# zacz08/ADM

Hardware: AMD Instinct MI355X
Metric: train images/sec (CIFAR-10 32x32 uncond DDM UNet, 1 optimizer step/iter) + 10-step sample images/sec (higher is better)
Workload: dtype f32; 1 GPU; BASELINE configs[1]: CIFAR-10 32x32 uncond two-decoder DhariwalUNet (216M params), bs=128/GPU fp32, ddm_const schedule, dropout 0.1, loss_simple (LPIPS term needs unfetchable VGG16 weights), clip 1.0 + AdamW + EMA(every 8); global_batch=128, image=3x32x32, parallelism=dp1, valid=True

## Files before the change

adm_amd/csrc/conv_wino2d_x6.hip:

```cpp
#include "common.h"
#include "split_format.h"
#include <type_traits>

#ifndef X6_TL
#define X6_TL 0
#endif
#ifndef X6_SHARE
#define X6_SHARE 0
#endif
#ifndef X6_ABL
#define X6_ABL 0
#endif

namespace {

struct X6P {
  const float* x; const unsigned short* w; const float* bias; const float* res; float* y;
  int Mt, N, H, W, Hh, Wh, Cin, ldx, ldy, ldr, wrows, tilesN, xbytes, wbytes, plane;
  int splitk, chunks_per_split; float* ws;
  int ybytes, rbytes;
  int up;
  const float* amax_x; float wscale;
};

typedef __attribute__((address_space(3))) void x6_lds_void;
constexpr int X6P_T = 64, X6N = 64, X6K = 16;
[[maybe_unused]] constexpr int X6_A_STAGE = 4 * 3 * X6P_T * X6K;
[[maybe_unused]] constexpr int X6_B_STAGE = 4 * 3 * X6N * X6K;
template <int FMT, int NB = 2> struct X6Fmt {
  static constexpr int TERMS = split_terms(FMT);
  static constexpr int NT = 32 * NB;
  static constexpr int CONS = 2 * NB;
  static constexpr int THREADS = (CONS + 4) * 64;
  static constexpr int A_STAGE = 4 * TERMS * X6P_T * X6K;
  static constexpr int B_STAGE = 4 * TERMS * NT * X6K;
  static constexpr int DMA_PER_WAVE = 2 * TERMS;
  static constexpr int RB = NB > 2 ? 3 : 4;
  static constexpr int PD = NB > 2 ? 3 : 4;
};
constexpr int X6_RA = 2;

__device__ __forceinline__ f32x4 sub4(f32x4 a, f32x4 b) { return a - b; }
__device__ __forceinline__ f32x16 sub16(f32x16 a, f32x16 b) { return a - b; }

__device__ __forceinline__ void h3_store(const f32x4 (&e)[4], unsigned short* la, float s) {
  if (X6_ABL & 2) return;
  const f32x4 v[4] = {plain_sub4(e[0], e[2]), plain_add4(e[1], e[2]), plain_sub4(e[2], e[1]), plain_sub4(e[1], e[3])};
#pragma unroll
  for (int ex = 0; ex < 4; ++ex) {
    u32x2 t0, t1;
    split2_quad(v[ex], s, t0, t1);
    *reinterpret_cast<u32x2*>(la + (ex * 2 + 0) * X6P_T * X6K) = t0;
    *reinterpret_cast<u32x2*>(la + (ex * 2 + 1) * X6P_T * X6K) = t1;
  }
}

__device__ __forceinline__ void x6_store(const f32x4 (&e)[4], unsigned short* la) {
  if (X6_ABL & 2) return;
  const f32x4 v[4] = {plain_sub4(e[0], e[2]), plain_add4(e[1], e[2]), plain_sub4(e[2], e[1]), plain_sub4(e[1], e[3])};
#pragma unroll
  for (int ex = 0; ex < 4; ++ex) {
    u32x2 t0, t1, t2;
    split3_quad(v[ex], t0, t1, t2);
    *reinterpret_cast<u32x2*>(la + (ex * 3 + 0) * X6P_T * X6K) = t0;
    *reinterpret_cast<u32x2*>(la + (ex * 3 + 1) * X6P_T * X6K) = t1;
    *reinterpret_cast<u32x2*>(la + (ex * 3 + 2) * X6P_T * X6K) = t2;
  }
}

#ifndef X6_KB_N
#define X6_KB_N 4
#endif
constexpr int X6_KB = X6_KB_N;
struct X6Seq {
  int k0, len, ey, cc, skip2;
  __device__ __forceinline__ void init(int chunks, int up) { k0 = 0; len = min(X6_KB, chunks); ey = 0; cc = 0; skip2 = up; }
  __device__ __forceinline__ int chunk() const { return k0 + cc; }
  __device__ __forceinline__ bool done() const { return len <= 0; }
  __device__ __forceinline__ void next(int chunks) {
    if (++cc == len) {
      cc = 0;
      ++ey;
      if (skip2 && ey == 2) ++ey;
      if (ey == 4) { ey = 0; k0 += len; len = min(X6_KB, chunks - k0); }
    }
  }
};

template <int FMT, int NB>
__global__ __launch_bounds__((2 * NB + 4) * 64) void wino2d_x6_kernel(X6P p) {
  using F = X6Fmt<FMT, NB>;
  constexpr int TERMS = F::TERMS;
  float sa = 1.f, inv_scale = 1.f;
  if (FMT) { sa = split_scale(adm_amax_read(p.amax_x)); inv_scale = 1.f / (sa * p.wscale); }
  extern __shared__ __attribute__((aligned(16))) unsigned short smem6[];
  unsigned short* As = smem6;
  unsigned short* Bs = smem6 + X6_RA * F::A_STAGE;
  const int tid = threadIdx.x, lane = tid & 63, hw_wid = tid >> 6;
  const bool producer = hw_wid >= F::CONS;
  const int wid = producer ? hw_wid - F::CONS : hw_wid;
  const int bid = adm_xcd_remap(blockIdx.x, gridDim.x);
  const int tilesM = gridDim.x / p.tilesN;
  const int tm = bid % tilesM, tn = bid / tilesM;
  const int mt0 = tm * X6P_T, n0 = tn * F::NT;
  constexpr unsigned OOB = 0x80000000u;

  const int c_begin = (p.splitk > 1) ? (int)blockIdx.y * p.chunks_per_split : 0;
  const int chunks = (p.splitk > 1) ? min(p.chunks_per_split, (p.Cin >> 4) - c_begin) : (p.Cin >> 4);
  const int S = (p.up ? 3 : 4) * chunks;

  if (producer) {
    const __amdgpu_buffer_rsrc_t rs_x = __builtin_amdgcn_make_buffer_rsrc(const_cast<float*>(p.x), 0, p.xbytes, 0x00020000);
    const int ptid = wid * 64 + lane;
    const int pl = ptid >> 2, aq = ptid & 3;
    unsigned a_base = 0, colmask = 0, rowmask = 0;
    bool take_l = false, take_r = false;
    {
      const int t = mt0 + pl;
      if (t < p.Mt) {
        const int xp = t % p.Wh;
        const int u = t / p.Wh;
        const int ty = u % p.Hh, b = u / p.Hh;
        a_base = p.up ? (unsigned)((((long)b * p.Hh + ty) * p.Wh + xp) * p.ldx + aq * 4) * 4u
                      : (unsigned)((((long)b * p.H + 2 * ty) * p.W + 2 * xp) * p.ldx + aq * 4) * 4u;
        colmask = (xp > 0 ? 1u : 0u) | 6u | (2 * xp + 2 < p.W ? 8u : 0u);
        rowmask = (ty > 0 ? 1u : 0u) | 6u | (2 * ty + 2 < p.H ? 8u : 0u);
        if (X6_SHARE && !p.up) {
          take_l = xp > 0 && (pl & 15) != 0;
          take_r = xp + 1 < p.Wh && (pl & 15) != 15 && t + 1 < p.Mt;
          if (take_l) colmask &= ~1u;
          if (take_r) colmask &= ~8u;
        }
      }
    }
    unsigned short* la = As + pl * X6K + ((((aq >> 1) ^ (pl >> 3)) & 1) << 3) + (aq & 1) * 4;
    X6Seq ld; ld.init(chunks, p.up);
    unsigned a_voff[2][4];
    int voff_ey = -1;
    auto set_rows = [&]() {
      const int ey = ld.ey;
      const int iA = (ey == 0) ? 0 : 1, iB = (ey == 3) ? 3 : 2;
      const bool live = !ld.done();
      const bool vA = ((rowmask >> iA) & 1u) && live, vB = ((rowmask >> iB) & 1u) && live;
      const int offA = (p.up ? ((iA + 1) >> 1) - 1 : iA - 1) * (p.up ? p.Wh : p.W) * p.ldx * 4;
      const int offB = (p.up ? ((iB + 1) >> 1) - 1 : iB - 1) * (p.up ? p.Wh : p.W) * p.ldx * 4;
#pragma unroll
      for (int j = 0; j < 4; ++j) {
        const bool cv = (colmask >> j) & 1u;
        const int cj = (p.up ? ((j + 1) >> 1) - 1 : j - 1) * p.ldx * 4;
        a_voff[0][j] = (vA && cv) ? a_base + (unsigned)(offA + cj) : OOB;
        a_voff[1][j] = (vB && cv) ? a_base + (unsigned)(offB + cj) : OOB;
      }
      voff_ey = live ? ey : 4;
    };
    constexpr int D = F::PD;
    f32x4 dA[D][4], dB[D][4];
    int set_ey[D];
    auto issue = [&](int d) {
      if (voff_ey != (ld.done() ? 4 : ld.ey)) set_rows();
      const int soff = (c_begin + ld.chunk()) << 6;
#pragma unroll
      for (int j = 0; j < 4; ++j) {
        if (X6_ABL & 1) { dA[d][j] = f32x4{1.f, 2.f, 3.f, (float)soff}; dB[d][j] = f32x4{0.5f, 0.25f, (float)j, 1.f}; continue; }
        dA[d][j] = __builtin_bit_cast(f32x4, __builtin_amdgcn_raw_buffer_load_b128(rs_x, (int)a_voff[0][j], soff, 0));
        dB[d][j] = __builtin_bit_cast(f32x4, __builtin_amdgcn_raw_buffer_load_b128(rs_x, (int)a_voff[1][j], soff, 0));
      }
      set_ey[d] = ld.ey;
      if (!ld.done()) ld.next(chunks);
    };
    auto store = [&](int d, int slot) {
      f32x4 e[4];
      if (set_ey[d] == 1) {
#pragma unroll
        for (int j = 0; j < 4; ++j) e[j] = plain_add4(dA[d][j], dB[d][j]);
      } else if (set_ey[d] == 2) {
#pragma unroll
        for (int j = 0; j < 4; ++j) e[j] = plain_sub4(dB[d][j], dA[d][j]);
      } else {
#pragma unroll
        for (int j = 0; j < 4; ++j) e[j] = plain_sub4(dA[d][j], dB[d][j]);
      }
      if (X6_SHARE && !p.up) {
        f32x4 el, er;
#pragma unroll
        for (int i = 0; i < 4; ++i) { el[i] = __shfl_up(e[2][i], 4, 64); er[i] = __shfl_down(e[1][i], 4, 64); }
        if (take_l) e[0] = el;
        if (take_r) e[3] = er;
      }
      if (FMT) h3_store(e, la + slot * F::A_STAGE, sa);
      else x6_store(e, la + slot * F::A_STAGE);
    };
#pragma unroll
    for (int d = 0; d < D; ++d) issue(d);
    __builtin_amdgcn_sched_barrier(0);
    constexpr int TRIP = (D & 1) ? 2 * D : D;
    for (int t = 0; t < S; t += TRIP) {
#pragma unroll
      for (int k = 0; k < TRIP; ++k) {
        const int d = k % D;
        if (t + k < S) {
          const bool tl = X6_TL && p.ws && blockIdx.x == 0 && tid == F::CONS * 64 && t + k < 48;
          unsigned long long* TL = reinterpret_cast<unsigned long long*>(p.ws) + 1024 + (t + k) * 4;
          if (tl) TL[0] = __builtin_readcyclecounter();
          store(d, k & 1);
          __builtin_amdgcn_sched_barrier(0);
          if (tl) { asm volatile("s_waitcnt lgkmcnt(0)" ::: "memory"); TL[1] = __builtin_readcyclecounter(); }
          issue(d);
          __builtin_amdgcn_sched_barrier(0);
          if (tl) TL[2] = __builtin_readcyclecounter();
          adm_lds_barrier();
          if (tl) TL[3] = __builtin_readcyclecounter();
        }
      }
    }
    return;
  }

  const __amdgpu_buffer_rsrc_t rs_w = __builtin_amdgcn_make_buffer_rsrc(const_cast<unsigned short*>(p.w), 0, p.wbytes, 0x00020000);
  const int wm = wid / NB, wn = wid % NB;
  const int lr = lane & 31, lh = lane >> 5;
  if (p.splitk > 1) {
    p.y = p.ws + (long)blockIdx.y * ((long)p.Mt * 4) * p.N;
    p.ldy = p.N; p.bias = nullptr; p.res = nullptr;
    const long sb = (long)p.Mt * 4 * p.N * 4;
    p.ybytes = sb < (1L << 31) ? (int)sb : 0;
  }
  constexpr int QW = F::DMA_PER_WAVE;
  unsigned b_voff[QW];
#pragma unroll
  for (int i = 0; i < QW; ++i) {
    const int q = wid * QW + i, pt = q / NB;
    const int row = (q % NB) * 32 + (lane >> 1);
    const int n = n0 + row;
    const int half = (lane ^ (row >> 3)) & 1;
    b_voff[i] = (n < p.wrows) ? (unsigned)((((long)pt * p.wrows + n) * 16 + half * 8) * 2) : OOB;
  }
  X6Seq lb; lb.init(chunks, p.up);
  int ld_slot = 0;
  auto issue_b = [&]() {
    const int kb = ((lb.ey * (p.Cin >> 4) + c_begin + lb.chunk()) * (4 * TERMS) * p.wrows) << 5;
    unsigned short* dst = Bs + ld_slot * F::B_STAGE + (wid * QW) * 512;
    if (!(X6_ABL & 4)) {
#pragma unroll
      for (int i = 0; i < QW; ++i)
        __builtin_amdgcn_raw_ptr_buffer_load_lds(rs_w, (x6_lds_void*)(dst + i * 512), 16, (int)b_voff[i], kb, 0, 0);
    }
    lb.next(chunks);
    if (++ld_slot == F::RB) ld_slot = 0;
  };

  f32x16 acc[4];
  f32x16 Y[2][2];
#pragma unroll
  for (int a = 0; a < 2; ++a)
#pragma unroll
    for (int b = 0; b < 2; ++b)
#pragma unroll
      for (int r = 0; r < 16; ++r) Y[a][b][r] = 0.f;
  const int a_foff = (wm * 32 + lr) * X6K + ((lh ^ (lr >> 3)) & 1) * 8;
  const int b_foff = (wn * 32 + lr) * X6K + ((lh ^ (lr >> 3)) & 1) * 8;
  const f32x16 zero = {0.f, 0.f, 0.f, 0.f, 0.f, 0.f, 0.f, 0.f, 0.f, 0.f, 0.f, 0.f, 0.f, 0.f, 0.f, 0.f};

  X6Seq cs; cs.init(chunks, p.up);
  int slot_b = 0;
#pragma unroll
  for (int i = 0; i < F::RB - 1; ++i) issue_b();
  for (int t = 0; t < S; ++t) {
    const bool tl = X6_TL && p.ws && blockIdx.x == 0 && tid == 0 && t < 48;
    unsigned long long* TL = reinterpret_cast<unsigned long long*>(p.ws) + t * 4;
    if (tl) TL[0] = __builtin_readcyclecounter();
    if (F::RB == 4 && t + 2 < S) { if (FMT) asm volatile("s_waitcnt vmcnt(8) lgkmcnt(0)\n\ts_barrier" ::: "memory"); else asm volatile("s_waitcnt vmcnt(12) lgkmcnt(0)\n\ts_barrier" ::: "memory"); }
    else if (t + 1 < S) { if (FMT) asm volatile("s_waitcnt vmcnt(4) lgkmcnt(0)\n\ts_barrier" ::: "memory"); else asm volatile("s_waitcnt vmcnt(6) lgkmcnt(0)\n\ts_barrier" ::: "memory"); }
    else asm volatile("s_waitcnt vmcnt(0) lgkmcnt(0)\n\ts_barrier" ::: "memory");
    if (tl) TL[1] = __builtin_readcyclecounter();
    if (t + F::RB - 1 < S) issue_b();
    const unsigned short* Ab = As + (t & 1) * F::A_STAGE + a_foff;
    const unsigned short* Bb = Bs + slot_b * F::B_STAGE + b_foff;
    if (++slot_b == F::RB) slot_b = 0;
    const bool first = cs.cc == 0;
    u32x4 fa[NB > 2 ? 1 : 2][TERMS], fb[NB > 2 ? 1 : 2][TERMS];
    auto frag = [&](int xi, int set) {
#pragma unroll
      for (int k = 0; k < TERMS; ++k) {
        if (X6_ABL & 16) {
          fa[set][k] = u32x4{0x3f803f80u, (unsigned)t, 0x3f803f80u, (unsigned)xi};
          fb[set][k] = u32x4{0x3f003f00u, (unsigned)k, 0x3f003f00u, (unsigned)lane};
          continue;
        }
        fa[set][k] = *reinterpret_cast<const u32x4*>(Ab + (xi * TERMS + k) * X6P_T * X6K);
        fb[set][k] = *reinterpret_cast<const u32x4*>(Bb + (xi * TERMS + k) * F::NT * X6K);
      }
    };
    auto products = [&](auto first_tag) {
      if (NB > 2) {
#pragma unroll
        for (int xi = 0; xi < 4; ++xi) {
          frag(xi, 0);
          if (X6_ABL & 8) continue;
          const f16x8 a0 = __builtin_bit_cast(f16x8, fa[0][0]), a1 = __builtin_bit_cast(f16x8, fa[0][1]);
          const f16x8 b0 = __builtin_bit_cast(f16x8, fb[0][0]), b1 = __builtin_bit_cast(f16x8, fb[0][1]);
          f32x16 c;
          if (decltype(first_tag)::value) asm volatile("v_mfma_f32_32x32x16_f16 %0, %1, %2, 0" : "=&v"(c) : "v"(a0), "v"(b1));
          else c = __builtin_amdgcn_mfma_f32_32x32x16_f16(a0, b1, acc[xi], 0, 0, 0);
          c = __builtin_amdgcn_mfma_f32_32x32x16_f16(a1, b0, c, 0, 0, 0);
          acc[xi] = __builtin_amdgcn_mfma_f32_32x32x16_f16(a0, b0, c, 0, 0, 0);
        }
        return;
      }
      frag(0, 0);
#pragma unroll
      for (int xi = 0; xi < 4; ++xi) {
        const int cur = xi & 1;
        if (xi < 3) frag(xi + 1, cur ^ 1);
        __builtin_amdgcn_sched_barrier(0);
        if (X6_ABL & 8) continue;
        const f32x16 c0 = decltype(first_tag)::value ? zero : acc[xi];
// ... 107 lines not shown
      p.y[px * p.ldy + n] = y0;
      p.y[(px + 1) * p.ldy + n] = y1;
    }
  }
}

__global__ void split3_kernel(const float* __restrict__ src, unsigned short* __restrict__ dst, int rows, int cols) {
  const long per = (long)rows * cols, total = per * 16;
  for (long i = blockIdx.x * (long)blockDim.x + threadIdx.x; i < total; i += (long)gridDim.x * blockDim.x) {
    const int img = (int)(i / per);
    const long rc = i - img * per;
    const int n = (int)(rc / cols), c = (int)(rc - (long)n * cols);
    split3_store(src[i], dst + wino_image_offset(3, img >> 2, img & 3, rows, cols, n, c), split_term_stride(rows));
  }
}

__global__ void split2_kernel(const float* __restrict__ src, unsigned short* __restrict__ dst, int rows, int cols, float scale,
                              int* __restrict__ overflow) {
  const long per = (long)rows * cols, total = per * 16;
  bool bad = false;
  for (long i = blockIdx.x * (long)blockDim.x + threadIdx.x; i < total; i += (long)gridDim.x * blockDim.x) {
    const int img = (int)(i / per);
    const long rc = i - img * per;
    const int n = (int)(rc / cols), c = (int)(rc - (long)n * cols);
    const float a = src[i] * scale;
    bad |= split_f16_overflow(a);
    split2_store(a, dst + wino_image_offset(2, img >> 2, img & 3, rows, cols, n, c), split_term_stride(rows));
  }
  if (bad && overflow) *overflow = 1;
}

}

extern "C" int adm_split3_bf16(const float* src, void* dst, int rows, int cols, hipStream_t stream) {
  if (!src || !dst || rows <= 0 || cols <= 0 || (cols & 15)) return ADM_EINVAL;
  const long total = (long)rows * cols * 16;
  const int grid = (int)((total + 255) / 256 > 4096 ? 4096 : (total + 255) / 256);
  hipLaunchKernelGGL(split3_kernel, dim3(grid), dim3(256), 0, stream, src, static_cast<unsigned short*>(dst), rows, cols);
  ADM_CHECK_LAUNCH();
  return ADM_OK;
}

extern "C" int adm_split2_f16(const float* src, void* dst, int rows, int cols, float scale, int* overflow, hipStream_t stream) {
  if (!src || !dst || rows <= 0 || cols <= 0 || (cols & 15) || !(scale > 0.f)) return ADM_EINVAL;
  const long total = (long)rows * cols * 16;
  const int grid = (int)((total + 255) / 256 > 4096 ? 4096 : (total + 255) / 256);
  hipLaunchKernelGGL(split2_kernel, dim3(grid), dim3(256), 0, stream, src, static_cast<unsigned short*>(dst), rows, cols, scale, overflow);
  ADM_CHECK_LAUNCH();
  return ADM_OK;
}

static int g_h3_wide = -1;
extern "C" int adm_wino2d_h3_wide(int v) { const int old = g_h3_wide; g_h3_wide = v; return old; }

static int wino2d_x6_launch(const float* x, const void* wq6, const float* bias, const float* res, float* y, float* ws, long ws_floats,
                            int B, int H, int W, int Cin, int ldx, int N, int wrows, int ldy, int ldr, int up, hipStream_t stream,
                            const float* amax_x = nullptr, float wscale = 0.f) {
  const bool h3 = amax_x != nullptr;
  if (!x || !wq6 || !y || B <= 0 || H < 2 || W < 2 || (W & 1) || (H & 1)) return ADM_EINVAL;
  if ((Cin & 31) || (ldx & 3) || N <= 0 || wrows < N) return ADM_EINVAL;
  if (((uintptr_t)x | (uintptr_t)wq6) & 15) return ADM_EINVAL;
  X6P p;
  p.x = x; p.w = static_cast<const unsigned short*>(wq6); p.bias = bias; p.res = res; p.y = y;
  const long Mt = (long)B * (H / 2) * (W / 2);
  const long xb = (long)B * H * W * ldx * 4 / (up ? 4 : 1), wb = (h3 ? 32L : 48L) * wrows * Cin * 2;
  if (h3 && !(wscale > 0.f)) return ADM_EINVAL;
  if (Mt >= (1L << 30) || xb >= (1L << 31) || wb >= (1L << 31)) return ADM_EINVAL;
  p.Mt = (int)Mt; p.N = N; p.H = H; p.W = W; p.Hh = H / 2; p.Wh = W / 2; p.Cin = Cin; p.ldx = ldx; p.ldy = ldy; p.ldr = ldr;
  p.wrows = wrows; p.xbytes = (int)xb; p.wbytes = (int)wb; p.plane = wrows * Cin; p.up = up ? 1 : 0;
  p.amax_x = amax_x; p.wscale = wscale;
  p.tilesN = adm_cdiv(N, X6N);
  const long mtiles = adm_cdiv(Mt, X6P_T);
  p.splitk = 1; p.chunks_per_split = 0; p.ws = X6_TL ? ws : nullptr;
  const long yb = (long)B * H * W * ldy * 4, rb = res ? (long)B * H * W * ldr * 4 : 0;
  p.ybytes = (yb < (1L << 31) && rb < (1L << 31)) ? (int)yb : 0;
  p.rbytes = (int)rb;
  const int sk = (ws && !(N & 3) && !(ldy & 3) && (!res || !(ldr & 3))) ? adm_wino2d_x6_splitk(B, H, W, Cin, N) : 1;
  if (sk > 1 && ws_floats >= (long)sk * Mt * 4 * N) {
    const int chunks = Cin >> 4;
    p.chunks_per_split = ((chunks + sk - 1) / sk + 1) & ~1;
    p.splitk = (chunks + p.chunks_per_split - 1) / p.chunks_per_split;
    p.ws = ws;
  }
  constexpr int smem0 = (X6_RA * X6Fmt<0>::A_STAGE + X6Fmt<0>::RB * X6Fmt<0>::B_STAGE) * (int)sizeof(unsigned short);
  constexpr int smem1 = (X6_RA * X6Fmt<1>::A_STAGE + X6Fmt<1>::RB * X6Fmt<1>::B_STAGE) * (int)sizeof(unsigned short);
  constexpr int smemw = (X6_RA * X6Fmt<1, 4>::A_STAGE + X6Fmt<1, 4>::RB * X6Fmt<1, 4>::B_STAGE) * (int)sizeof(unsigned short);
  constexpr int smem3 = (X6_RA * X6Fmt<1, 3>::A_STAGE + X6Fmt<1, 3>::RB * X6Fmt<1, 3>::B_STAGE) * (int)sizeof(unsigned short);
  static bool attr_set = false;
  if (!attr_set) {
    if (hipFuncSetAttribute(reinterpret_cast<const void*>(&wino2d_x6_kernel<0, 2>), hipFuncAttributeMaxDynamicSharedMemorySize, smem0) != hipSuccess ||
        hipFuncSetAttribute(reinterpret_cast<const void*>(&wino2d_x6_kernel<1, 2>), hipFuncAttributeMaxDynamicSharedMemorySize, smem1) != hipSuccess ||
        hipFuncSetAttribute(reinterpret_cast<const void*>(&wino2d_x6_kernel<1, 4>), hipFuncAttributeMaxDynamicSharedMemorySize, smemw) != hipSuccess ||
        hipFuncSetAttribute(reinterpret_cast<const void*>(&wino2d_x6_kernel<1, 3>), hipFuncAttributeMaxDynamicSharedMemorySize, smem3) != hipSuccess)
      return ADM_ELAUNCH;
    attr_set = true;
  }
  int form = 2;
  if (h3 && p.splitk == 1 && g_h3_wide != 0 && N > X6N) {
    if (g_h3_wide == 1) form = 4;
    else if (g_h3_wide == 3) form = 3;
    else {
      const long cost[3] = {48, 60, 64};
      long best = -1;
      for (int nb = 2; nb <= 4; ++nb) {
        const long t = (mtiles * adm_cdiv(N, 32 * nb) + 255) / 256 * cost[nb - 2];
        if (best < 0 || t < best) { best = t; form = nb; }
      }
    }
  }
  const bool three = form == 3, wide = form == 4;
  if (three) {
    p.tilesN = adm_cdiv(N, X6Fmt<1, 3>::NT);
    hipLaunchKernelGGL((wino2d_x6_kernel<1, 3>), dim3((unsigned)(mtiles * p.tilesN), 1), dim3(X6Fmt<1, 3>::THREADS), smem3, stream, p);
  } else if (wide) {
    p.tilesN = adm_cdiv(N, X6Fmt<1, 4>::NT);
    hipLaunchKernelGGL((wino2d_x6_kernel<1, 4>), dim3((unsigned)(mtiles * p.tilesN), 1), dim3(X6Fmt<1, 4>::THREADS), smemw, stream, p);
  } else if (h3) {
    hipLaunchKernelGGL((wino2d_x6_kernel<1, 2>), dim3((unsigned)(mtiles * p.tilesN), p.splitk), dim3(512), smem1, stream, p);
  } else {
    hipLaunchKernelGGL((wino2d_x6_kernel<0, 2>), dim3((unsigned)(mtiles * p.tilesN), p.splitk), dim3(512), smem0, stream, p);
  }
  ADM_CHECK_LAUNCH();
  if (p.splitk > 1) return adm_splitk_reduce(ws, bias, res, y, Mt * 4, N, ldy, ldr, p.splitk, stream);
  return ADM_OK;
}

extern "C" int adm_conv_fwd_wino2d_h3(const float* x, const void* wqh, const float* bias, const float* res, float* y, float* ws,
                                      long ws_floats, int B, int H, int W, int Cin, int ldx, int N, int wrows, int ldy, int ldr,
                                      const float* amax_x, float wscale, int up, hipStream_t stream) {
  if (!amax_x) return ADM_EINVAL;
  return wino2d_x6_launch(x, wqh, bias, res, y, ws, ws_floats, B, H, W, Cin, ldx, N, wrows, ldy, ldr, up, stream, amax_x, wscale);
}

extern "C" int adm_conv_fwd_wino2d_x6(const float* x, const void* wq6, const float* bias, const float* res, float* y, float* ws,
                                      long ws_floats, int B, int H, int W, int Cin, int ldx, int N, int wrows, int ldy, int ldr,
                                      hipStream_t stream) {
  return wino2d_x6_launch(x, wq6, bias, res, y, ws, ws_floats, B, H, W, Cin, ldx, N, wrows, ldy, ldr, 0, stream);
}

extern "C" int adm_conv_fwd_wino2d_x6_up(const float* x, const void* wq6, const float* bias, const float* res, float* y, float* ws,
                                         long ws_floats, int B, int H, int W, int Cin, int ldx, int N, int wrows, int ldy, int ldr,
                                         hipStream_t stream) {
  return wino2d_x6_launch(x, wq6, bias, res, y, ws, ws_floats, B, H, W, Cin, ldx, N, wrows, ldy, ldr, 1, stream);
}

extern "C" int adm_wino2d_x6_splitk(int B, int H, int W, int Cin, int N) {
  const long wgs = (long)adm_cdiv((long)B * (H / 2) * (W / 2), X6P_T) * adm_cdiv(N, X6N);
  const int chunks = Cin >> 4;
  if (wgs >= 192 || chunks < 8) return 1;
  int best = 1;
  long best_t = (wgs + 255) / 256 * (4L * chunks + 12);
  for (int s = 2; s <= 6 && s <= chunks / 4; ++s) {
    const int cps = ((chunks + s - 1) / s + 1) & ~1;
    const int splits = (chunks + cps - 1) / cps;
    const long t = (wgs * splits + 255) / 256 * (4L * cps + 12);
    if (t < best_t) { best_t = t; best = s; }
  }
  return best;
}
```

adm_amd/hip.py:

```python
from __future__ import annotations

import ctypes
import os
import subprocess
from ctypes import c_double, c_float, c_int, c_long, c_uint64, c_void_p

import torch

_HERE = os.path.dirname(os.path.abspath(__file__))
LIB_PATH = os.path.join(_HERE, "libadm_hip.so")
_lib = None

P, I, L, F, D, U = c_void_p, c_int, c_long, c_float, c_double, c_uint64
_SIGS = {
    "adm_version": [],
    "adm_conv_fwd": [P, P, P, P, P, I, I, I, I, I, I, I, I, I, I, I, I, P],
    "adm_conv_splitk": [I, I, I],
    "adm_conv_fwd_ws": [P, P, P, P, P, P, L, I, I, I, I, I, I, I, I, I, I, I, P],
    "adm_conv_fwd_strided": [P, P, P, P, P, I, I, I, I, I, I, I, I, I, I, I, I, I, I, P],
    "adm_conv_fwd_wino": [P, P, P, P, P, I, I, I, I, I, I, I, I, I, P],
    "adm_conv_fwd_wino_up": [P, P, P, P, P, I, I, I, I, I, I, I, I, I, P],
    "adm_pack_weight_wino": [P, P, P, I, I, I, I, P],
    "adm_pack_weight_wino2d": [P, P, P, I, I, I, I, P],
    "adm_conv_fwd_wino2d": [P, P, P, P, P, P, L, I, I, I, I, I, I, I, I, I, P],
    "adm_wino2d_splitk": [I, I, I, I, I],
    "adm_wino2d_variant": [I],
    "adm_wino2d_h3_wide": [I],
    "adm_wgrad_h3_blocks": [I],
    "adm_conv_fwd_wino2d_x6": [P, P, P, P, P, P, L, I, I, I, I, I, I, I, I, I, P],
    "adm_conv_fwd_wino2d_x6_up": [P, P, P, P, P, P, L, I, I, I, I, I, I, I, I, I, P],
    "adm_wino2d_x6_splitk": [I, I, I, I, I],
    "adm_split3_bf16": [P, P, I, I, P],
    "adm_split2_f16": [P, P, I, I, F, P, P],
    "adm_conv_fwd_wino2d_h3": [P, P, P, P, P, P, L, I, I, I, I, I, I, I, I, I, P, F, I, P],
    "adm_gemm_x6": [P, P, P, P, P, L, I, I, I, I, I, I, P],
    "adm_gemm_x6_amax": [P, P, P, P, P, L, I, I, I, I, I, I, P, P],
    "adm_gemm_x6_h3": [P, P, P, P, P, L, I, I, I, I, I, I, P, F, P, P],
    "adm_split2_rows_f16": [P, P, I, I, I, F, P, P],
    "adm_split3_rows": [P, P, I, I, I, P],
    "adm_conv_wgrad_x6": [P, P, P, P, I, I, I, I, I, I, I, I, P],
    "adm_conv_wgrad_x6_up": [P, P, P, P, I, I, I, I, I, I, I, I, P],
    "adm_conv_wgrad_x6_ws": [P, P, P, P, I, I, I, I, I, I, I, I, I, P],
    "adm_conv_wgrad_x6_plan": [I, I, I, I, I],
    "adm_gemm_wgrad_x6": [P, P, P, P, L, I, I, I, I, I, P],
    "adm_gemm_wgrad_x6_ws": [P, P, P, P, L, I, I, I, I, I, P],
    "adm_gemm_wgrad_x6_plan": [L, I, I],
    "adm_conv_wgrad_x6_h3": [P, P, P, P, I, I, I, I, I, I, I, I, I, I, P, P, P],
    "adm_gemm_wgrad_x6_h3": [P, P, P, P, L, I, I, I, I, I, I, P, P, P],
    "adm_conv_wgrad_x6_bf16a": [P, P, P, P, I, I, I, I, I, I, I, I, I, P],
    "adm_gemm_wgrad_x6_bf16a": [P, P, P, P, L, I, I, I, I, I, P],
    "adm_conv_wgrad": [P, P, P, I, I, I, I, I, I, I, I, I, I, P],
    "adm_conv_wgrad_wino": [P, P, P, P, I, I, I, I, I, I, I, I, P],
    "adm_conv_wgrad_wino_up": [P, P, P, P, I, I, I, I, I, I, I, I, P],
    "adm_conv_wgrad_bias": [P, P, P, P, I, I, I, I, I, I, I, I, I, I, P],
    "adm_conv_wgrad_wino2d": [P, P, P, P, I, I, I, I, I, I, I, I, P],
    "adm_unpack_wgrad_wino2d": [P, I, P, I, I, I, I, I, P, P, P],
    "adm_conv_wgrad_plan": [I, I, I, I, I, I, I, I],
    "adm_conv_wgrad_ws": [P, P, P, P, I, I, I, I, I, I, I, I, I, I, I, P],
    "adm_unpack_wgrad_splits": [P, I, P, I, I, I, I, I, I, I, P, P, P],
    "adm_conv_fwd_bf16": [P, P, P, P, P, I, I, I, I, I, I, I, I, I, I, I, I, P],
    "adm_conv_wgrad_bf16": [P, P, P, I, I, I, I, I, I, I, I, I, I, P],
    "adm_conv_fwd_bf16a": [P, P, P, P, P, I, I, I, I, I, I, I, I, I, I, I, I, P],
    "adm_conv_wgrad_bf16a": [P, P, P, I, I, I, I, I, I, I, I, I, I, P],
    "adm_gn_fwd_bf16out": [P, P, P, P, P, P, L, P, I, I, I, I, F, I, F, U, P],
    "adm_f32_to_bf16": [P, P, L, P],
    "adm_conv_bf16_tile": [L, I],
    "adm_conv_wgrad_bf16_plan": [L, I, I, I, I, P],
    "adm_pack_weight": [P, P, P, I, I, I, I, I, I, P],
    "adm_pack_weight_table": [P, I, L, P],
    "adm_unpack_wgrad_table": [P, I, L, P],
    "adm_gn_bwd_param_table": [P, I, L, P],
    "adm_unpack_wgrad": [P, P, I, I, I, I, I, I, I, P],
    "adm_permute_vec": [P, P, I, I, I, I, P],
    "adm_colsum": [P, P, I, I, I, I, P],
    "adm_gn_splits": [I, I],
    "adm_gn_fused": [I],
    "adm_gn_plan": [I, I, I, P],
    "adm_gn_stats": [P, P, P, I, I, I, I, F, P],
    "adm_gn_apply": [P, P, P, P, P, L, P, I, I, I, I, I, F, U, P],
    "adm_gn_fwd": [P, P, P, P, P, P, L, P, I, I, I, I, F, I, F, U, P],
# ... 98 lines not shown
    "adm_ln_affine_bwd": [P, P, P, P, P, P, P, L, I, F, I, P],
    "adm_swin_merge_ln_bwd": [P, P, P, P, P, P, P, I, I, I, I, F, I, P],
    "adm_rowscale_add": [P, P, P, P, I, L, P],
    "adm_patch_embed_ln_fwd": [P, P, P, P, P, P, I, I, I, I, F, P],
    "adm_patch_embed_ln_bwd_ws_floats": [I, I, I, I],
    "adm_patch_embed_ln_bwd": [P, P, P, P, P, P, P, P, P, P, I, I, I, I, F, I, P],
    "adm_sr_tile": [I],
    "adm_sr_batch": [P, L, P, P, I, P, P, P, P, P, P, I, P, P, I, P, P, P, I, I, I, I, I, P],
    "adm_inpaint_masks": [P, P, P, P, P, P, P, P, P, I, I, P],
    "adm_inpaint_batch": [P, L, P, P, I, P, P, P, P, P, P, P, P, P, P, I, I, P],
    "adm_inpaint_compose": [P, P, P, P, I, I, L, P],
    "adm_pair_resize_lds": [I, I, I, I, I, I],
    "adm_pair_resize_batch": [P, L, P, P, P, L, P, P, I, P, L, P, I, P, I, I, I, I, P, P, P, P, P, P, I, I, I, P],
    "adm_image_resize_batch": [P, L, P, P, I, I, P, L, P, I, P, I, I, I, I, P, P, P, P, I, I, I, P],
    "adm_conv_rect_relu_fwd": [P, P, P, P, I, I, I, I, I, I, I, I, I, I, I, I, I, I, I, P],
    "adm_pool3x3_fwd": [P, P, I, I, I, I, I, I, I, I, P],
    "adm_global_avgpool_fwd": [P, P, I, I, I, I, I, P],
    "adm_tf1_resize_norm_u8": [P, P, I, I, I, P],
    "adm_feat_stats_accum": [P, I, I, P, P, P, I, P],
    "adm_depth_batch": [P, L, P, P, P, L, P, P, I, I, I, I, I, P, P, P, P, P, P, I, I, I, P],
    "adm_depth_metrics_blocks": [L],
    "adm_depth_metrics": [P, P, P, P, P, I, L, D, D, P],
    "adm_kid_sums_tile": [I],
    "adm_kid_sums_blocks": [I],
    "adm_kid_sums": [P, I, P, I, I, P, P, I, I, I, D, D, P, P, P],
}
EXPORTS = tuple(_SIGS)


def build(verbose: bool = False) -> str:
    r = subprocess.run(["make", "-C", os.path.join(_HERE, "csrc"), "-j8"], capture_output=True, text=True)
    if verbose or r.returncode != 0:
        print(r.stdout[-4000:], r.stderr[-8000:])
    if r.returncode != 0 or not os.path.exists(LIB_PATH):
        raise RuntimeError("building libadm_hip.so failed")
    return LIB_PATH


def lib() -> ctypes.CDLL:
    global _lib
    if _lib is None:
        if not os.path.exists(LIB_PATH):
            raise RuntimeError(f"{LIB_PATH} is missing: run `python -c 'import __graft_entry__ as g; g.build()'` "
                               "(there is no non-HIP fallback for the adm_amd hot path)")
        _lib = ctypes.CDLL(LIB_PATH)
        for name, args in _SIGS.items():
            fn = getattr(_lib, name)
            fn.argtypes = args
            fn.restype = c_long if name in ("adm_aug_workspace_floats", "adm_linattn_ws_floats", "adm_swin_attn_bwd_ws_floats",
                                        "adm_ln_bwd_ws_floats", "adm_pair_resize_lds", "adm_patch_embed_ln_bwd_ws_floats",
                                        "adm_kid_sums_blocks") else c_int
        if os.environ.get("ADM_H3_WIDE") is not None:
            _lib.adm_wino2d_h3_wide(int(os.environ["ADM_H3_WIDE"]))
        if os.environ.get("ADM_WGRAD_H3_BLOCKS") is not None:
            _lib.adm_wgrad_h3_blocks(int(os.environ["ADM_WGRAD_H3_BLOCKS"]))
    return _lib


def stream() -> c_void_p:
    return c_void_p(torch.cuda.current_stream().cuda_stream)


def ptr(t) -> c_void_p:
    return None if t is None else c_void_p(t.data_ptr())


NO_STREAM = ("adm_version", "adm_conv_splitk", "adm_gn_splits", "adm_aug_workspace_floats", "adm_conv_wgrad_plan",
             "adm_sumsq_blocks", "adm_lnc_blocks", "adm_bn_blocks", "adm_linattn_ws_floats", "adm_wino2d_splitk", "adm_wino2d_x6_splitk", "adm_wino2d_variant", "adm_wino2d_h3_wide", "adm_wgrad_h3_blocks", "adm_gn_fused", "adm_gn_plan", "adm_conv_wgrad_x6_plan", "adm_gemm_wgrad_x6_plan", "adm_lpips_head_blocks", "adm_ae_blocks", "adm_swin_attn_bwd_ws_floats", "adm_ln_bwd_ws_floats", "adm_sr_tile", "adm_pair_resize_lds", "adm_patch_embed_ln_bwd_ws_floats", "adm_conv_bf16_tile", "adm_conv_wgrad_bf16_plan", "adm_depth_metrics_blocks", "adm_kid_sums_tile", "adm_kid_sums_blocks")


def call(name: str, *args):
    rc = getattr(lib(), name)(*args, stream())
    if rc != 0:
        raise RuntimeError(f"{name} failed with code {rc} (-22 = unsupported shape/alignment, -5 = launch failure)")


def require_cuda(t: torch.Tensor, what: str = "tensor"):
    if not t.is_cuda:
        raise RuntimeError(f"adm_amd: {what} is on {t.device}; the HIP hot path needs a GPU tensor "
                           "(no CPU fallback exists by design)")
```

include/adm_hip.h:

```cpp
#ifndef ADM_HIP_H
#define ADM_HIP_H
#include <stdint.h>
typedef struct ihipStream_t* hipStream_t;

#ifdef __cplusplus
#define ADM_AMAX_SLOTS 64
#define ADM_AMAX_STRIDE 32
#define ADM_AMAX_FLOATS (ADM_AMAX_SLOTS * ADM_AMAX_STRIDE)

extern "C" {
#endif

int adm_version(void);


int adm_conv_fwd(const float* x, const float* wp, const float* bias, const float* res, float* y,
                 int B, int H, int W, int Cin, int ldx, int N, int wrows, int ldy, int ldr,
                 int ks, int up, int tile, hipStream_t stream);

int adm_conv_fwd_strided(const float* x, const float* wp, const float* bias, const float* res, float* y,
                         int B, int Hin, int Win, int Hout, int Wout, int Cin, int ldx, int N, int wrows,
                         int ldy, int ldr, int ks, int stride, int pad_lo, hipStream_t stream);

int adm_conv_fwd_wino(const float* x, const float* wq, const float* bias, const float* res, float* y, int B, int H, int W,
// ... 14 lines not shown
                        int Cout, int lddy, int ks, int up, int splits, hipStream_t stream);

int adm_conv_wgrad_wino(const float* x, const float* dy, float* dwp, float* dbias, int B, int H, int W, int Cin, int ldx,
                        int Cout, int lddy, int splits, hipStream_t stream);

int adm_conv_wgrad_wino_up(const float* x, const float* dy, float* dwp, float* dbias, int B, int H, int W, int Cin, int ldx,
                           int Cout, int lddy, int splits, hipStream_t stream);

int adm_pack_weight_wino2d(const float* w, float* wf, float* wb, int Co, int Ci, int Co_pad, int Ci_pad, hipStream_t stream);
int adm_conv_fwd_wino2d(const float* x, const float* wq, const float* bias, const float* res, float* y, float* ws, long ws_floats,
                        int B, int H, int W, int Cin, int ldx, int N, int wrows, int ldy, int ldr, hipStream_t stream);
int adm_conv_fwd_wino2d_x6(const float* x, const void* wq6, const float* bias, const float* res, float* y, float* ws,
                           long ws_floats, int B, int H, int W, int Cin, int ldx, int N, int wrows, int ldy, int ldr,
                           hipStream_t stream);
int adm_conv_fwd_wino2d_x6_up(const float* x, const void* wq6, const float* bias, const float* res, float* y, float* ws,
                              long ws_floats, int B, int H, int W, int Cin, int ldx, int N, int wrows, int ldy, int ldr,
                              hipStream_t stream);
int adm_wino2d_x6_splitk(int B, int H, int W, int Cin, int N);
int adm_split2_f16(const float* src, void* dst, int rows, int cols, float scale, int* overflow, hipStream_t stream);
int adm_conv_fwd_wino2d_h3(const float* x, const void* wqh, const float* bias, const float* res, float* y, float* ws,
                           long ws_floats, int B, int H, int W, int Cin, int ldx, int N, int wrows, int ldy, int ldr,
                           const float* amax_x, float wscale, int up, hipStream_t stream);
int adm_split3_bf16(const float* src, void* dst, int rows, int cols, hipStream_t stream);
int adm_gemm_x6(const float* x, const void* w6, const float* bias, const float* res, float* y, long M, int K, int ldx, int N, int wrows,
                int ldy, int ldr, hipStream_t stream);
int adm_split3_rows(const float* src, void* dst, int rows, int cols, int ld, hipStream_t stream);
int adm_gemm_x6_amax(const float* x, const void* w6, const float* bias, const float* res, float* y, long M, int K, int ldx, int N,
                     int wrows, int ldy, int ldr, float* amax_y, hipStream_t stream);
int adm_gemm_x6_h3(const float* x, const void* wh, const float* bias, const float* res, float* y, long M, int K, int ldx, int N, int wrows,
                   int ldy, int ldr, const float* amax_x, float wscale, float* amax_y, hipStream_t stream);
int adm_split2_rows_f16(const float* src, void* dst, int rows, int cols, int ld, float scale, int* overflow, hipStream_t stream);
int adm_conv_wgrad_x6(const float* x, const float* dy, float* dwp2, float* dbias, int B, int H, int W, int Cin, int ldx, int Cout,
                      int lddy, int splits, hipStream_t stream);
int adm_conv_wgrad_x6_up(const float* x, const float* dy, float* dwp2, float* dbias, int B, int H, int W, int Cin, int ldx, int Cout,
                         int lddy, int splits, hipStream_t stream);
int adm_conv_wgrad_x6_ws(const float* x, const float* dy, float* ws, float* bws, int B, int H, int W, int Cin, int ldx, int Cout,
                         int lddy, int splits, int up, hipStream_t stream);
int adm_conv_wgrad_x6_plan(int B, int H, int W, int Cin, int Cout);
int adm_gemm_wgrad_x6(const float* x, const float* dy, float* dwp, float* dbias, long P, int Cin, int ldx, int Cout, int lddy,
                      int splits, hipStream_t stream);
int adm_gemm_wgrad_x6_ws(const float* x, const float* dy, float* ws, float* bws, long P, int Cin, int ldx, int Cout, int lddy,
                         int splits, hipStream_t stream);
int adm_gemm_wgrad_x6_plan(long P, int Cin, int Cout);
int adm_conv_wgrad_x6_bf16a(const void* x16, const float* dy, float* dwp2, float* dbias, int B, int H, int W, int Cin, int ldx,
                            int Cout, int lddy, int splits, int up, hipStream_t stream);
int adm_gemm_wgrad_x6_bf16a(const void* x16, const float* dy, float* dwp, float* dbias, long P, int Cin, int ldx, int Cout, int lddy,
                            int splits, hipStream_t stream);
int adm_conv_wgrad_x6_h3(const float* x, const float* dy, float* dwp2, float* dbias, int B, int H, int W, int Cin, int ldx, int Cout,
                         int lddy, int splits, int up, int det, const float* amax_x, const float* amax_dy, hipStream_t stream);
int adm_gemm_wgrad_x6_h3(const float* x, const float* dy, float* dwp, float* dbias, long P, int Cin, int ldx, int Cout, int lddy,
                         int splits, int det, const float* amax_x, const float* amax_dy, hipStream_t stream);
int adm_wino2d_variant(int ws);
int adm_wino2d_h3_wide(int v);
int adm_wgrad_h3_blocks(int v);
int adm_wino2d_splitk(int B, int H, int W, int Cin, int N);

int adm_conv_wgrad_wino2d(const float* x, const float* dy, float* dwp2, float* dbias, int B, int H, int W, int Cin, int ldx,
                          int Cout, int lddy, int splits, hipStream_t stream);
int adm_unpack_wgrad_wino2d(const float* wx, int splits, float* dw, int Co, int Ci, int Co_pad, int Ci_pad, int accumulate,
                            const float* bws, float* dbias, hipStream_t stream);

int adm_conv_wgrad_plan(int B, int H, int W, int Cin, int Cout, int ks, int up, int wino);
int adm_conv_wgrad_ws(const float* x, const float* dy, float* ws, float* bws, int B, int H, int W, int Cin, int ldx, int Cout,
                      int lddy, int ks, int up, int splits, int wino, hipStream_t stream);

int adm_conv_fwd_bf16(const float* x, const unsigned short* wp16, const float* bias, const float* res, float* y,
                      int B, int H, int W, int Cin, int ldx, int N, int wrows, int ldy, int ldr, int ks, int up,
                      int tile, hipStream_t stream);
int adm_conv_wgrad_bf16(const float* x, const float* dy, float* dwp, int B, int H, int W, int Cin, int ldx, int Cout,
                        int lddy, int ks, int up, int splits, hipStream_t stream);
int adm_conv_fwd_bf16a(const void* x16, const unsigned short* wp16, const float* bias, const float* res, float* y, int B, int H, int W,
                       int Cin, int ldx, int N, int wrows, int ldy, int ldr, int ks, int up, int tile, hipStream_t stream);
int adm_conv_wgrad_bf16a(const void* x16, const float* dy, float* dwp, int B, int H, int W, int Cin, int ldx, int Cout, int lddy, int ks,
                         int up, int splits, hipStream_t stream);
int adm_gn_fwd_bf16out(const float* x, float* stats, double* ws, const float* gamma, const float* beta, const float* ss,
                       long ss_bstride, void* y16, int B, int HW, int C, int G, float eps, int silu, float drop_p, uint64_t seed,
                       hipStream_t stream);
int adm_f32_to_bf16(const float* src, unsigned short* dst, long n, hipStream_t stream);
int adm_conv_bf16_tile(long M, int N);
int adm_conv_wgrad_bf16_plan(long P, int Cin, int Cout, int ks, int splits, int* out);

int adm_pack_weight(const float* w, float* wp_fwd, float* wp_bwd, int Co, int Ci, int ks, int Co_pad, int Ci_pad,
                    int qkv, hipStream_t stream);
int adm_pack_weight_table(const long* table, int n_entries, long total_tiles, hipStream_t stream);
int adm_unpack_wgrad(const float* dwp, float* dw, int Co, int Ci, int ks, int Co_pad, int Ci_pad, int qkv,
                     int accumulate, hipStream_t stream);
int adm_unpack_wgrad_splits(const float* ws, int splits, float* dw, int Co, int Ci, int ks, int Co_pad, int Ci_pad, int qkv,
                            int accumulate, const float* bws, float* dbias, hipStream_t stream);
int adm_unpack_wgrad_table(const long* table, int rows, long total_blocks, hipStream_t stream);
int adm_permute_vec(const float* in, float* out, int n, int n_pad, int qkv, int inverse, hipStream_t stream);
int adm_colsum(const float* a, float* out, int M, int N, int ld, int accumulate, hipStream_t stream);


int adm_gn_fused(int on);
int adm_gn_splits(int HW, int C);
int adm_gn_plan(int HW, int C, int G, int* out);
int adm_gn_stats(const float* x, float* stats, double* ws, int B, int HW, int C, int G, float eps, hipStream_t stream);
int adm_gn_apply(const float* x, const float* stats, const float* gamma, const float* beta, const float* ss,
                 long ss_bstride, float* y, int B, int HW, int C, int G, int silu, float drop_p, uint64_t seed,
                 hipStream_t stream);
int adm_gn_fwd(const float* x, float* stats, double* ws, const float* gamma, const float* beta, const float* ss,
               long ss_bstride, float* y, int B, int HW, int C, int G, float eps, int silu, float drop_p, uint64_t seed,
               hipStream_t stream);
int adm_gn_fwd_amax(const float* x, float* stats, double* ws, const float* gamma, const float* beta, const float* ss,
                    long ss_bstride, float* y, float* amax, int B, int HW, int C, int G, float eps, int silu, float drop_p,
                    uint64_t seed, hipStream_t stream);
// ... 307 lines not shown
```

Measured before the change: 1274 images/s.

## Reuse loaded input rows across Winograd row transforms in x6 producer

Adds a row-reuse path to the Winograd 2D x6 forward producer for non-upsample convs. Each input row is loaded once and kept in registers across the four row-transform steps of a chunk block, replacing the generic per-step paths that reload two rows every step. This is meant to cut redundant global/buffer loads. It also removes the unused X6_SHARE shuffle path, makes the K-block size a template parameter, and adds a runtime toggle (on by default). The price is more templated kernel instances and a larger unrolled producer loop that may raise register pressure.

Result: faster. 1293 images/s (median of 6 runs) (+1.5%).

```diff
diff --git a/adm_amd/csrc/conv_wino2d_x6.hip b/adm_amd/csrc/conv_wino2d_x6.hip
--- a/adm_amd/csrc/conv_wino2d_x6.hip
+++ b/adm_amd/csrc/conv_wino2d_x6.hip
@@ -5,8 +5,8 @@
 #ifndef X6_TL
 #define X6_TL 0
 #endif
-#ifndef X6_SHARE
-#define X6_SHARE 0
+#ifndef X6_KB_N
+#define X6_KB_N 4
 #endif
 #ifndef X6_ABL
 #define X6_ABL 0
@@ -37,6 +37,7 @@
   static constexpr int DMA_PER_WAVE = 2 * TERMS;
   static constexpr int RB = NB > 2 ? 3 : 4;
   static constexpr int PD = NB > 2 ? 3 : 4;
+  static constexpr int KB = NB > 2 ? 3 : X6_KB_N;
 };
 constexpr int X6_RA = 2;
 
@@ -68,13 +69,9 @@
   }
 }
 
-#ifndef X6_KB_N
-#define X6_KB_N 4
-#endif
-constexpr int X6_KB = X6_KB_N;
-struct X6Seq {
+template <int KB> struct X6Seq {
   int k0, len, ey, cc, skip2;
-  __device__ __forceinline__ void init(int chunks, int up) { k0 = 0; len = min(X6_KB, chunks); ey = 0; cc = 0; skip2 = up; }
+  __device__ __forceinline__ void init(int chunks, int up, int start = 0) { k0 = start; len = min(KB, chunks - start); ey = 0; cc = 0; skip2 = up; }
   __device__ __forceinline__ int chunk() const { return k0 + cc; }
   __device__ __forceinline__ bool done() const { return len <= 0; }
   __device__ __forceinline__ void next(int chunks) {
@@ -82,14 +79,15 @@
       cc = 0;
       ++ey;
       if (skip2 && ey == 2) ++ey;
-      if (ey == 4) { ey = 0; k0 += len; len = min(X6_KB, chunks - k0); }
+      if (ey == 4) { ey = 0; k0 += len; len = min(KB, chunks - k0); }
     }
   }
 };
 
-template <int FMT, int NB>
+template <int FMT, int NB, int REUSE>
 __global__ __launch_bounds__((2 * NB + 4) * 64) void wino2d_x6_kernel(X6P p) {
   using F = X6Fmt<FMT, NB>;
+  using Seq = X6Seq<F::KB>;
   constexpr int TERMS = F::TERMS;
   float sa = 1.f, inv_scale = 1.f;
   if (FMT) { sa = split_scale(adm_amax_read(p.amax_x)); inv_scale = 1.f / (sa * p.wscale); }
@@ -114,7 +112,6 @@
     const int ptid = wid * 64 + lane;
     const int pl = ptid >> 2, aq = ptid & 3;
     unsigned a_base = 0, colmask = 0, rowmask = 0;
-    bool take_l = false, take_r = false;
     {
       const int t = mt0 + pl;
       if (t < p.Mt) {
@@ -125,16 +122,83 @@
                       : (unsigned)((((long)b * p.H + 2 * ty) * p.W + 2 * xp) * p.ldx + aq * 4) * 4u;
         colmask = (xp > 0 ? 1u : 0u) | 6u | (2 * xp + 2 < p.W ? 8u : 0u);
         rowmask = (ty > 0 ? 1u : 0u) | 6u | (2 * ty + 2 < p.H ? 8u : 0u);
-        if (X6_SHARE && !p.up) {
-          take_l = xp > 0 && (pl & 15) != 0;
-          take_r = xp + 1 < p.Wh && (pl & 15) != 15 && t + 1 < p.Mt;
-          if (take_l) colmask &= ~1u;
-          if (take_r) colmask &= ~8u;
+      }
+    }
+    unsigned short* la = As + pl * X6K + ((((aq >> 1) ^ (pl >> 3)) & 1) << 3) + (aq & 1) * 4;
+    constexpr int D = F::PD;
+    f32x4 dA[D][4], dB[D][4];
+    auto combine = [&](int ey, const f32x4 (&a)[4], const f32x4 (&b)[4], f32x4 (&e)[4]) {
+      if (ey == 1) {
+#pragma unroll
+        for (int j = 0; j < 4; ++j) e[j] = plain_add4(a[j], b[j]);
+      } else if (ey == 2) {
+#pragma unroll
+        for (int j = 0; j < 4; ++j) e[j] = plain_sub4(b[j], a[j]);
+      } else {
+#pragma unroll
+        for (int j = 0; j < 4; ++j) e[j] = plain_sub4(a[j], b[j]);
+      }
+    };
+    int k_done = 0, t_done = 0;
+    if constexpr (REUSE != 0 && F::KB == D) {
+      constexpr int KB = F::KB;
+      const int nwhole = p.up ? 0 : chunks / KB;
+      if (nwhole > 0) {
+        const int rstride = p.W * p.ldx * 4;
+        unsigned v0[4], vc[4];
+#pragma unroll
+        for (int j = 0; j < 4; ++j) {
+          const bool cv = (colmask >> j) & 1u;
+          const int cj = (j - 1) * p.ldx * 4;
+          vc[j] = cv ? a_base + (unsigned)cj : OOB;
+          v0[j] = (cv && (rowmask & 1u)) ? a_base + (unsigned)(cj - rstride) : OOB;
         }
-      }
-    }
-    unsigned short* la = As + pl * X6K + ((((aq >> 1) ^ (pl >> 3)) & 1) << 3) + (aq & 1) * 4;
-    X6Seq ld; ld.init(chunks, p.up);
+        const unsigned k3 = (rowmask & 8u) ? 0u : OOB;
+        auto row = [&](f32x4 (&dst)[4], const unsigned (&vo)[4], unsigned kill, int soff) {
+#pragma unroll
+          for (int j = 0; j < 4; ++j) {
+            if (X6_ABL & 1) { dst[j] = f32x4{1.f, 2.f, (float)j, (float)soff}; continue; }
+            dst[j] = __builtin_bit_cast(f32x4, __builtin_amdgcn_raw_buffer_load_b128(rs_x, (int)(vo[j] | kill), soff, 0));
+          }
+        };
+#pragma unroll
+        for (int cc = 0; cc < KB; ++cc) {
+          row(dA[cc], v0, 0u, (c_begin + cc) << 6);
+          row(dB[cc], vc, 0u, ((c_begin + cc) << 6) + rstride);
+          __builtin_amdgcn_sched_barrier(0);
+        }
+        for (int blk = 0; blk < nwhole; ++blk) {
+          const int cb = (c_begin + blk * KB) << 6;
+          const unsigned nx = blk + 1 < nwhole ? 0u : OOB;
+#pragma unroll
+          for (int ey = 0; ey < 4; ++ey) {
+#pragma unroll
+            for (int cc = 0; cc < KB; ++cc) {
+              const int k = ey * KB + cc, ts = blk * 4 * KB + k;
+              const bool tl = X6_TL && p.ws && blockIdx.x == 0 && tid == F::CONS * 64 && ts < 48;
+              unsigned long long* TL = reinterpret_cast<unsigned long long*>(p.ws) + 1024 + ts * 4;
+              if (tl) TL[0] = __builtin_readcyclecounter();
+              f32x4 e[4];
+              combine(ey, dA[cc], dB[cc], e);
+              if (FMT) h3_store(e, la + (k & 1) * F::A_STAGE, sa);
+              else x6_store(e, la + (k & 1) * F::A_STAGE);
+              __builtin_amdgcn_sched_barrier(0);
+              if (tl) { asm volatile("s_waitcnt lgkmcnt(0)" ::: "memory"); TL[1] = __builtin_readcyclecounter(); }
+              const int so = cb + (cc << 6);
+              if (ey == 0) row(dA[cc], vc, 0u, so);
+              if (ey == 2) row(dB[cc], vc, k3, so + 2 * rstride);
+              if (ey == 3) { row(dA[cc], v0, nx, so + (KB << 6)); row(dB[cc], vc, nx, so + (KB << 6) + rstride); }
+              __builtin_amdgcn_sched_barrier(0);
+              if (tl) TL[2] = __builtin_readcyclecounter();
+              adm_lds_barrier();
+              if (tl) TL[3] = __builtin_readcyclecounter();
+            }
+          }
+        }
+        k_done = nwhole * KB; t_done = nwhole * 4 * KB;
+      }
+    }
+    Seq ld; ld.init(chunks, p.up, k_done);
     unsigned a_voff[2][4];
     int voff_ey = -1;
     auto set_rows = [&]() {
@@ -153,8 +217,6 @@
       }
       voff_ey = live ? ey : 4;
     };
-    constexpr int D = F::PD;
-    f32x4 dA[D][4], dB[D][4];
     int set_ey[D];
     auto issue = [&](int d) {
       if (voff_ey != (ld.done() ? 4 : ld.ey)) set_rows();
@@ -170,37 +232,23 @@
     };
     auto store = [&](int d, int slot) {
       f32x4 e[4];
-      if (set_ey[d] == 1) {
-#pragma unroll
-        for (int j = 0; j < 4; ++j) e[j] = plain_add4(dA[d][j], dB[d][j]);
-      } else if (set_ey[d] == 2) {
-#pragma unroll
-        for (int j = 0; j < 4; ++j) e[j] = plain_sub4(dB[d][j], dA[d][j]);
-      } else {
-#pragma unroll
-        for (int j = 0; j < 4; ++j) e[j] = plain_sub4(dA[d][j], dB[d][j]);
-      }
-      if (X6_SHARE && !p.up) {
-        f32x4 el, er;
-#pragma unroll
-        for (int i = 0; i < 4; ++i) { el[i] = __shfl_up(e[2][i], 4, 64); er[i] = __shfl_down(e[1][i], 4, 64); }
-        if (take_l) e[0] = el;
-        if (take_r) e[3] = er;
-      }
+      combine(set_ey[d], dA[d], dB[d], e);
       if (FMT) h3_store(e, la + slot * F::A_STAGE, sa);
       else x6_store(e, la + slot * F::A_STAGE);
     };
+    const int S_gen = S - t_done;
+    if (S_gen <= 0) return;
 #pragma unroll
     for (int d = 0; d < D; ++d) issue(d);
     __builtin_amdgcn_sched_barrier(0);
     constexpr int TRIP = (D & 1) ? 2 * D : D;
-    for (int t = 0; t < S; t += TRIP) {
+    for (int t = 0; t < S_gen; t += TRIP) {
 #pragma unroll
       for (int k = 0; k < TRIP; ++k) {
         const int d = k % D;
-        if (t + k < S) {
-          const bool tl = X6_TL && p.ws && blockIdx.x == 0 && tid == F::CONS * 64 && t + k < 48;
-          unsigned long long* TL = reinterpret_cast<unsigned long long*>(p.ws) + 1024 + (t + k) * 4;
+        if (t + k < S_gen) {
+          const bool tl = X6_TL && p.ws && blockIdx.x == 0 && tid == F::CONS * 64 && t_done + t + k < 48;
+          unsigned long long* TL = reinterpret_cast<unsigned long long*>(p.ws) + 1024 + (t_done + t + k) * 4;
           if (tl) TL[0] = __builtin_readcyclecounter();
           store(d, k & 1);
           __builtin_amdgcn_sched_barrier(0);
@@ -235,7 +283,7 @@
     const int half = (lane ^ (row >> 3)) & 1;
     b_voff[i] = (n < p.wrows) ? (unsigned)((((long)pt * p.wrows + n) * 16 + half * 8) * 2) : OOB;
   }
-  X6Seq lb; lb.init(chunks, p.up);
+  Seq lb; lb.init(chunks, p.up);
   int ld_slot = 0;
   auto issue_b = [&]() {
     const int kb = ((lb.ey * (p.Cin >> 4) + c_begin + lb.chunk()) * (4 * TERMS) * p.wrows) << 5;
@@ -261,7 +309,7 @@
   const int b_foff = (wn * 32 + lr) * X6K + ((lh ^ (lr >> 3)) & 1) * 8;
   const f32x16 zero = {0.f, 0.f, 0.f, 0.f, 0.f, 0.f, 0.f, 0.f, 0.f, 0.f, 0.f, 0.f, 0.f, 0.f, 0.f, 0.f};
 
-  X6Seq cs; cs.init(chunks, p.up);
+  Seq cs; cs.init(chunks, p.up);
   int slot_b = 0;
 #pragma unroll
   for (int i = 0; i < F::RB - 1; ++i) issue_b();
@@ -475,6 +523,23 @@
 
 static int g_h3_wide = -1;
 extern "C" int adm_wino2d_h3_wide(int v) { const int old = g_h3_wide; g_h3_wide = v; return old; }
+static int g_row_reuse = 1;
+extern "C" int adm_wino2d_x6_row_reuse(int v) { const int old = g_row_reuse; if (v >= 0) g_row_reuse = v ? 1 : 0; return old; }
+
+template <int FMT, int NB> static int x6_launch_form(const X6P& p, unsigned gx, unsigned gy, hipStream_t stream) {
+  using F = X6Fmt<FMT, NB>;
+  constexpr int smem = (X6_RA * F::A_STAGE + F::RB * F::B_STAGE) * (int)sizeof(unsigned short);
+  static bool attr_set = false;
+  if (!attr_set) {
+    if (hipFuncSetAttribute(reinterpret_cast<const void*>(&wino2d_x6_kernel<FMT, NB, 1>), hipFuncAttributeMaxDynamicSharedMemorySize, smem) != hipSuccess ||
+        hipFuncSetAttribute(reinterpret_cast<const void*>(&wino2d_x6_kernel<FMT, NB, 0>), hipFuncAttributeMaxDynamicSharedMemorySize, smem) != hipSuccess)
+      return ADM_ELAUNCH;
+    attr_set = true;
+  }
+  if (g_row_reuse) hipLaunchKernelGGL((wino2d_x6_kernel<FMT, NB, 1>), dim3(gx, gy), dim3(F::THREADS), smem, stream, p);
+  else hipLaunchKernelGGL((wino2d_x6_kernel<FMT, NB, 0>), dim3(gx, gy), dim3(F::THREADS), smem, stream, p);
+  return ADM_OK;
+}
 
 static int wino2d_x6_launch(const float* x, const void* wq6, const float* bias, const float* res, float* y, float* ws, long ws_floats,
                             int B, int H, int W, int Cin, int ldx, int N, int wrows, int ldy, int ldr, int up, hipStream_t stream,
@@ -505,19 +570,6 @@
     p.splitk = (chunks + p.chunks_per_split - 1) / p.chunks_per_split;
     p.ws = ws;
   }
-  constexpr int smem0 = (X6_RA * X6Fmt<0>::A_STAGE + X6Fmt<0>::RB * X6Fmt<0>::B_STAGE) * (int)sizeof(unsigned short);
-  constexpr int smem1 = (X6_RA * X6Fmt<1>::A_STAGE + X6Fmt<1>::RB * X6Fmt<1>::B_STAGE) * (int)sizeof(unsigned short);
-  constexpr int smemw = (X6_RA * X6Fmt<1, 4>::A_STAGE + X6Fmt<1, 4>::RB * X6Fmt<1, 4>::B_STAGE) * (int)sizeof(unsigned short);
-  constexpr int smem3 = (X6_RA * X6Fmt<1, 3>::A_STAGE + X6Fmt<1, 3>::RB * X6Fmt<1, 3>::B_STAGE) * (int)sizeof(unsigned short);
-  static bool attr_set = false;
-  if (!attr_set) {
-    if (hipFuncSetAttribute(reinterpret_cast<const void*>(&wino2d_x6_kernel<0, 2>), hipFuncAttributeMaxDynamicSharedMemorySize, smem0) != hipSuccess ||
-        hipFuncSetAttribute(reinterpret_cast<const void*>(&wino2d_x6_kernel<1, 2>), hipFuncAttributeMaxDynamicSharedMemorySize, smem1) != hipSuccess ||
-        hipFuncSetAttribute(reinterpret_cast<const void*>(&wino2d_x6_kernel<1, 4>), hipFuncAttributeMaxDynamicSharedMemorySize, smemw) != hipSuccess ||
-        hipFuncSetAttribute(reinterpret_cast<const void*>(&wino2d_x6_kernel<1, 3>), hipFuncAttributeMaxDynamicSharedMemorySize, smem3) != hipSuccess)
-      return ADM_ELAUNCH;
-    attr_set = true;
-  }
   int form = 2;
   if (h3 && p.splitk == 1 && g_h3_wide != 0 && N > X6N) {
     if (g_h3_wide == 1) form = 4;
@@ -531,18 +583,19 @@
       }
     }
   }
-  const bool three = form == 3, wide = form == 4;
-  if (three) {
+  int rc;
+  if (form == 3) {
     p.tilesN = adm_cdiv(N, X6Fmt<1, 3>::NT);
-    hipLaunchKernelGGL((wino2d_x6_kernel<1, 3>), dim3((unsigned)(mtiles * p.tilesN), 1), dim3(X6Fmt<1, 3>::THREADS), smem3, stream, p);
-  } else if (wide) {
+    rc = x6_launch_form<1, 3>(p, (unsigned)(mtiles * p.tilesN), 1, stream);
+  } else if (form == 4) {
     p.tilesN = adm_cdiv(N, X6Fmt<1, 4>::NT);
-    hipLaunchKernelGGL((wino2d_x6_kernel<1, 4>), dim3((unsigned)(mtiles * p.tilesN), 1), dim3(X6Fmt<1, 4>::THREADS), smemw, stream, p);
+    rc = x6_launch_form<1, 4>(p, (unsigned)(mtiles * p.tilesN), 1, stream);
   } else if (h3) {
-    hipLaunchKernelGGL((wino2d_x6_kernel<1, 2>), dim3((unsigned)(mtiles * p.tilesN), p.splitk), dim3(512), smem1, stream, p);
+    rc = x6_launch_form<1, 2>(p, (unsigned)(mtiles * p.tilesN), (unsigned)p.splitk, stream);
   } else {
-    hipLaunchKernelGGL((wino2d_x6_kernel<0, 2>), dim3((unsigned)(mtiles * p.tilesN), p.splitk), dim3(512), smem0, stream, p);
-  }
+    rc = x6_launch_form<0, 2>(p, (unsigned)(mtiles * p.tilesN), (unsigned)p.splitk, stream);
+  }
+  if (rc != ADM_OK) return rc;
   ADM_CHECK_LAUNCH();
   if (p.splitk > 1) return adm_splitk_reduce(ws, bias, res, y, Mt * 4, N, ldy, ldr, p.splitk, stream);
   return ADM_OK;
diff --git a/adm_amd/hip.py b/adm_amd/hip.py
--- a/adm_amd/hip.py
+++ b/adm_amd/hip.py
@@ -26,6 +26,7 @@
     "adm_wino2d_splitk": [I, I, I, I, I],
     "adm_wino2d_variant": [I],
     "adm_wino2d_h3_wide": [I],
+    "adm_wino2d_x6_row_reuse": [I],
     "adm_wgrad_h3_blocks": [I],
     "adm_conv_fwd_wino2d_x6": [P, P, P, P, P, P, L, I, I, I, I, I, I, I, I, I, P],
     "adm_conv_fwd_wino2d_x6_up": [P, P, P, P, P, P, L, I, I, I, I, I, I, I, I, I, P],
@@ -230,6 +231,8 @@
                                         "adm_kid_sums_blocks") else c_int
         if os.environ.get("ADM_H3_WIDE") is not None:
             _lib.adm_wino2d_h3_wide(int(os.environ["ADM_H3_WIDE"]))
+        if os.environ.get("ADM_X6_ROW_REUSE") is not None:
+            _lib.adm_wino2d_x6_row_reuse(int(os.environ["ADM_X6_ROW_REUSE"]))
         if os.environ.get("ADM_WGRAD_H3_BLOCKS") is not None:
             _lib.adm_wgrad_h3_blocks(int(os.environ["ADM_WGRAD_H3_BLOCKS"]))
     return _lib
@@ -244,7 +247,7 @@
 
 
 NO_STREAM = ("adm_version", "adm_conv_splitk", "adm_gn_splits", "adm_aug_workspace_floats", "adm_conv_wgrad_plan",
-             "adm_sumsq_blocks", "adm_lnc_blocks", "adm_bn_blocks", "adm_linattn_ws_floats", "adm_wino2d_splitk", "adm_wino2d_x6_splitk", "adm_wino2d_variant", "adm_wino2d_h3_wide", "adm_wgrad_h3_blocks", "adm_gn_fused", "adm_gn_plan", "adm_conv_wgrad_x6_plan", "adm_gemm_wgrad_x6_plan", "adm_lpips_head_blocks", "adm_ae_blocks", "adm_swin_attn_bwd_ws_floats", "adm_ln_bwd_ws_floats", "adm_sr_tile", "adm_pair_resize_lds", "adm_patch_embed_ln_bwd_ws_floats", "adm_conv_bf16_tile", "adm_conv_wgrad_bf16_plan", "adm_depth_metrics_blocks", "adm_kid_sums_tile", "adm_kid_sums_blocks")
+             "adm_sumsq_blocks", "adm_lnc_blocks", "adm_bn_blocks", "adm_linattn_ws_floats", "adm_wino2d_splitk", "adm_wino2d_x6_splitk", "adm_wino2d_variant", "adm_wino2d_h3_wide", "adm_wino2d_x6_row_reuse", "adm_wgrad_h3_blocks", "adm_gn_fused", "adm_gn_plan", "adm_conv_wgrad_x6_plan", "adm_gemm_wgrad_x6_plan", "adm_lpips_head_blocks", "adm_ae_blocks", "adm_swin_attn_bwd_ws_floats", "adm_ln_bwd_ws_floats", "adm_sr_tile", "adm_pair_resize_lds", "adm_patch_embed_ln_bwd_ws_floats", "adm_conv_bf16_tile", "adm_conv_wgrad_bf16_plan", "adm_depth_metrics_blocks", "adm_kid_sums_tile", "adm_kid_sums_blocks")
 
 
 def call(name: str, *args):
diff --git a/include/adm_hip.h b/include/adm_hip.h
--- a/include/adm_hip.h
+++ b/include/adm_hip.h
@@ -90,6 +90,7 @@
                          int splits, int det, const float* amax_x, const float* amax_dy, hipStream_t stream);
 int adm_wino2d_variant(int ws);
 int adm_wino2d_h3_wide(int v);
+int adm_wino2d_x6_row_reuse(int v);
 int adm_wgrad_h3_blocks(int v);
 int adm_wino2d_splitk(int B, int H, int W, int Cin, int N);
 
```
